# davek44/Glimmer-MG

Measured on AMD Instinct MI355X. Metric: Mbases/s scored (6-frame IMM), higher is better.
Workload: dtype f64

## Files before the change

### glimmer-mg_amd/build.py

```python
import fcntl
import os
import shutil
import subprocess

PKG = os.path.dirname(os.path.abspath(__file__))
LIB = os.path.join(PKG, "lib", "libgmg.so")
SOURCES = ["csrc/gmg_api.hip", "csrc/gmg_kernels.hip", "csrc/gmg_frame6.hip", "csrc/gmg_orfs.hip", "csrc/gmg_mg.hip", "csrc/gmg_ingest.hip", "csrc/gmg_strings.hip", "csrc/gmg_train.hip", "csrc/gmg_fixed.hip", "csrc/gmg_tophits.hip", "csrc/gmg_models.hip", "csrc/gmg_entropy.hip", "csrc/gmg_extract.hip", "csrc/gmg_features.hip", "host/icm.cc", "host/icm_train.cc", "host/fixed_icm.cc", "host/gmg_icm_c.cc", "host/gmg_shard.cc", "host/gmg_classes.cc", "host/gmg_extract_plan.cc", "host/gmg_features_host.cc"]
HEADERS = ["csrc/gmg_internal.h", "csrc/gmg_device.h", "csrc/gmg_scan.h", "csrc/gmg_mg_errtile.h", "csrc/gmg_mg_errwave.h", "csrc/gmg_mg_orfbits.h", "csrc/gmg_mg_run.h", "host/icm.hh", "host/icm_internal.hh", "../include/gmg.h", "../include/gmg_icm.h"]
FLAGS = ["--offload-arch=gfx950", "-O3", "-std=c++17", "-fPIC", "-shared", "-ffp-contract=off",
         "-Wall", "-Wno-unused-function"]


def stale():
    if not os.path.exists(LIB):
        return True
    t = os.path.getmtime(LIB)
    return any(os.path.getmtime(os.path.join(PKG, f)) > t for f in SOURCES + HEADERS)


def build_variant(name, defines):
    hipcc = shutil.which("hipcc") or "/opt/rocm/bin/hipcc"
    out = os.path.join(PKG, "lib", "variants", "libgmg_%s.so" % name)
    os.makedirs(os.path.dirname(out), exist_ok=True)
    cmd = [hipcc, *FLAGS, *["-D" + d for d in defines], "-o", out, *SOURCES]
    res = subprocess.run(cmd, cwd=PKG, stdout=subprocess.PIPE, stderr=subprocess.STDOUT, text=True)
    if res.returncode != 0:
        print(res.stdout)
        raise RuntimeError("hipcc failed building " + out)
    return out

# ... 77 lines not shown
```

### glimmer-mg_amd/capi.py

```python
import ctypes as C
import os

from .build import LIB

_lib = None

vp = C.c_void_p
u64 = C.c_uint64
i32 = C.c_int


class Segment(C.Structure):
    _fields_ = [("read", C.c_uint32), ("lo", C.c_uint32), ("len", C.c_uint32), ("orient", C.c_uint32)]


class GeneRegion(C.Structure):
    _fields_ = [("read", C.c_uint32), ("first", C.c_int32), ("len", C.c_int32), ("strand", C.c_int32)]


class Coord(C.Structure):
    _fields_ = [("read", C.c_uint32), ("dir", C.c_int32), ("start", C.c_int64), ("end", C.c_int64)]


class FeatureGene(C.Structure):
# ... 52 lines not shown
    "gmg_icm_bytes_info": (i32, [vp, u64, C.POINTER(i32), C.POINTER(i32), C.POINTER(i32), C.POINTER(i32), C.POINTER(u64)]),
    "gmg_model_set_load": (i32, [vp, vp, i32, C.POINTER(vp), vp]),
    "gmg_model_set_finish": (i32, [vp, C.POINTER(i32)]),
    "gmg_model_set_model": (vp, [vp, i32]),
    "gmg_model_set_free": (i32, [vp]),
    "gmg_model_blob": (i32, [vp, vp, C.POINTER(C.c_size_t)]),
    "gmg_model_value_stats": (i32, [vp, C.POINTER(i32), C.POINTER(i32), C.POINTER(i32)]),
    "gmg_reads_upload": (i32, [vp, vp, u64, C.POINTER(vp)]),
    "gmg_reads_wrap_device": (i32, [vp, vp, u64, u64, C.POINTER(vp)]),
    "gmg_reads_free": (i32, [vp]),
    "gmg_reads_info": (i32, [vp, C.POINTER(u64), C.POINTER(u64)]),
    "gmg_reads_download": (i32, [vp, vp, vp]),
    "gmg_reads_select": (i32, [vp, vp, u64, C.POINTER(vp)]),
    "gmg_reads_extract": (i32, [vp, vp, u64, i32, vp, vp, u64, C.POINTER(vp)]),
    "gmg_fasta_ambiguous": (i32, [C.c_char_p, u64, vp, vp, u64, C.POINTER(u64)]),
    "gmg_extract_plan": (i32, [vp, u64, vp, u64, i32, C.c_int64, vp, vp, C.POINTER(u64)]),
    "gmg_single_create": (i32, [C.POINTER(vp)]),
    "gmg_single_stage": (i32, [vp, C.c_char_p, u64, i32, C.POINTER(vp), C.POINTER(vp), C.POINTER(vp)]),
    "gmg_single_fetch": (i32, [vp, vp, C.c_size_t]),
    "gmg_single_free": (i32, [vp]),
    "gmg_single_window": (i32, [vp, vp, vp, i32, i32, vp, vp]),
    "gmg_segments_upload": (i32, [vp, vp, u64, vp, C.POINTER(u64), C.POINTER(vp)]),
    "gmg_segments_free": (i32, [vp]),
    "gmg_frame_score6": (i32, [vp, vp, vp, vp, vp]),
    "gmg_frame_score6_strided": (i32, [vp, vp, vp, vp, u64, vp]),
    "gmg_null_set_upload": (i32, [vp, i32, C.POINTER(vp)]),
    "gmg_null_set_from_tables": (i32, [vp, vp, i32, C.POINTER(vp)]),
    "gmg_null_set_build": (i32, [vp, i32, vp, i32, C.POINTER(vp)]),
    "gmg_null_set_free": (i32, [vp]),
    "gmg_frame_score6_nulls": (i32, [vp, vp, vp, vp, vp, u64, vp]),
    "gmg_segment_frame_score": (i32, [vp, vp, vp, i32, vp, vp]),
    "gmg_segment_cumscore": (i32, [vp, vp, vp, i32, vp, vp]),
    "gmg_score_string": (i32, [vp, vp, vp, i32, vp, vp]),
    "gmg_segment_partial_prob": (i32, [vp, vp, vp, i32, vp, vp]),
    "gmg_all_frame_score": (i32, [vp, vp, vp, vp, vp, vp, vp]),
    "gmg_window_distrib": (i32, [vp, vp, vp, u64, vp, vp, vp]),
    "gmg_mg_score_reads": (i32, [vp, vp, vp, vp, vp, C.POINTER(vp), vp]),
    "gmg_mg_score_groups": (i32, [vp, i32, vp, vp, vp, C.POINTER(vp), vp]),
    "gmg_find_orfs": (i32, [vp, vp, C.POINTER(vp), vp]),
    "gmg_mg_result_info": (i32, [vp, C.POINTER(u64), C.POINTER(u64)]),
    "gmg_mg_result_fetch": (i32, [vp, vp, vp, vp]),
    "gmg_mg_result_fetch_errors": (i32, [vp, vp]),
    "gmg_mg_result_free": (i32, [vp]),
    "gmg_trim_cache": (i32, []),
    "gmg_score_reads_strings": (i32, [vp, i32, vp, vp, vp]),
    "gmg_host_register": (i32, [vp, C.c_size_t]),
# ... 87 lines not shown
```

### glimmer-mg_amd/csrc/gmg_api.hip

```cpp

#include "gmg_internal.h"
#include "gmg_scan.h"

#include <ctype.h>
#include <stdarg.h>
#include <stdio.h>
#include <stdlib.h>
#include <string.h>
#include <new>
#include <mutex>
#include <vector>

static thread_local char g_err[512] = "";
static int g_device = -1;

int gmg_set_error(int code, const char *fmt, ...)
{
    va_list ap;
    va_start(ap, fmt);
    vsnprintf(g_err, sizeof g_err, fmt, ap);
    va_end(ap);
    return code;
}

extern "C" const char *gmg_last_error(void) { return g_err; }

long long g_gmg_opt[GMG_OPT_COUNT] = {
     0,  0,  0,  0,  0,  0,
     0,  -1,  0x7ffffffell,  0,  0,
     0,  0,  1,  1,  1,  1,  2,
     -1,  0,  1,  1,  0,  4,  0,  64ll << 20,  0,  0};
static const char *const g_opt_name[GMG_OPT_COUNT] = {
    "seg_plain", "mg_tile", "mg_one_stream", "mg_err_flat", "mg_err_calls", "mg_err_calls_grow", "orfs_exact_path",
    "train_sort_min", "mg_max_entries", "mg_timing", "ingest_timing", "train_timing", "diag", "strings_fused",
    "mg_gene32", "mg_fused", "mg_err_skip", "mg_orfs_events", "mg_err_tile", "mg_err_tile_q", "mg_err_qonly", "mg_err_wave", "mg_err_wave_q", "orfs_walk8", "ingest_scans", "ingest_piece_min", "mg_orfs_bits", "orfs_q_poison"};

static int opt_index(const char *key)
{
    for (int i = 0; key && i < GMG_OPT_COUNT; i++)
        if (strcmp(key, g_opt_name[i]) == 0) return i;
    return -1;
}

extern "C" int gmg_set_option(const char *key, long long value)
{
    const int i = opt_index(key);
    if (i < 0) return gmg_set_error(GMG_EINVAL, "gmg_set_option: unknown option '%s'", key ? key : "(null)");
#ifndef GMG_ABLATIONS
    if (i == GMG_OPT_DIAG && value != 0)
        return gmg_set_error(GMG_EINVAL, "gmg_set_option: the ablation kernels are not in this build (-DGMG_ABLATIONS)");
#endif
    if (i == GMG_OPT_MG_MAX_ENTRIES && (value < 1 || value > 0x7ffffffell))
        return gmg_set_error(GMG_EINVAL, "gmg_set_option: mg_max_entries must be in [1, 2^31 - 2]");
    g_gmg_opt[i] = value;
    return GMG_OK;
}

extern "C" int gmg_get_option(const char *key, long long *value)
// ... 1140 lines not shown
```

### glimmer-mg_amd/csrc/gmg_frame6.hip

```cpp

#include "gmg_device.h"
#include <stdlib.h>
#include <vector>

#ifndef GMG_F6_STAMPS
#define GMG_F6_STAMPS 0
#endif
#if GMG_F6_STAMPS
__device__ unsigned long long g_f6_stamps[1024 * 16 * 8];
extern "C" int gmg_debug_f6_stamps(unsigned long long *out, int n)
{
    return hipMemcpyFromSymbol(out, HIP_SYMBOL(g_f6_stamps), (size_t)n * 8) == hipSuccess ? 0 : -1;
}
#define F6_STAMP(i) do { const unsigned long long now_ = __builtin_readcyclecounter(); st_acc[i] += now_ - st_prev; st_prev = now_; } while (0)
#else
#define F6_STAMP(i) do { } while (0)
#endif

struct Frame6Args {
    GmgDevModel gene, nul;
    const uint32_t *packed;
    const uint64_t *off;
    const uint32_t *tile_read;
    uint64_t total, n_reads;
    uint64_t first, count;
    uint32_t p_blocks;
    double *out;
    uint64_t stride;
    float *out_gene;
    uint64_t gstride;
    double *str_sums;
    uint32_t uniform_len;
    const struct F6Round *rounds = nullptr;
    const GmgDevModel *gmodels = nullptr;
    const struct F6Range *ranges = nullptr;
    const uint64_t *group_read = nullptr;
    uint32_t n_rounds = 0, n_ranges = 0, n_groups = 0;
};
struct F6Round { uint32_t chunk0; uint32_t ng; };
#define F6_ROUND_N(r) ((r).ng & 31u)
#define F6_ROUND_GROUP(r) ((r).ng >> 5)
#define F6_MAX_GROUPS ((1 << 27) - 1)
struct F6Range { uint64_t first; uint32_t count, group; };

constexpr int f6_cstride(int dt) { return ((((1 << (2 * dt)) - 1) / 3) + 15) & ~15; }
constexpr int f6_level_base(int l) { return ((1 << (2 * l)) - 1) / 3; }

template <int CTRL, int ROW_MASK = 0xf>
__device__ __forceinline__ double f6_dpp_add(double x)
{
    const unsigned long long b = (unsigned long long)__double_as_longlong(x);
    const uint32_t lo = (uint32_t)__builtin_amdgcn_update_dpp(0, (int)(uint32_t)b, CTRL, ROW_MASK, 0xf, false);
    const uint32_t hi = (uint32_t)__builtin_amdgcn_update_dpp(0, (int)(uint32_t)(b >> 32), CTRL, ROW_MASK, 0xf, false);
    return x + __longlong_as_double((long long)((unsigned long long)hi << 32 | lo));
}
__device__ __forceinline__ double f6_row_sum(double x)
{
    x = f6_dpp_add<0xb1>(x);
    x = f6_dpp_add<0x4e>(x);
    x = f6_dpp_add<0x141>(x);
    x = f6_dpp_add<0x140>(x);
    return x;
}
__device__ __noinline__ void f6_sum_chunk_slow(double *sum, const int32_t *roff, uint32_t len, uint32_t len_magic, uint32_t rem0, int32_t wm1,
                                               uint32_t span0, uint32_t &rel_a, double f0, double r0, double f1, double r1)
{
    const uint32_t lane = threadIdx.x & 63u;
// ... 75 lines not shown
        const int32_t a0 = (int32_t)(ra * len) - (int32_t)rem0, a1 = a0 + (int32_t)len;
        if ((int32_t)span0 >= a0 + wm1 && (int32_t)span0 + 128 <= a1 - wm1) {
            rel_a = ra;
            const double f = f6_row_sum(f0 + f1), r = f6_row_sum(r0 + r1);
            if ((threadIdx.x & 15u) == 15u) { unsafeAtomicAdd(&sum[2 * ra], f); unsafeAtomicAdd(&sum[2 * ra + 1], r); }
            return;
        }
    }
    f6_sum_chunk_slow(sum, roff, len, len_magic, rem0, wm1, span0, rel_a, f0, r0, f1, r1);
}

template <int DT>
__device__ __forceinline__ uint32_t f6_descend(const uint8_t *tab, uint32_t C, uint32_t shift0)
{
    uint32_t idx = __builtin_amdgcn_ubfe(C, shift0, 2);
#pragma unroll
    for (int l = 1; l < DT; l++) {
        const uint32_t sh = tab[f6_level_base(l) + idx];
        idx = (idx << 2) | __builtin_amdgcn_ubfe(C, sh, 2);
    }
    return idx;
}

template <int BLOCK, int DT, int K, int DIAG, bool PAIR, bool GENE_ONLY, bool STRINGS = false, bool SUM = false, bool MULTI = false>
__global__ __launch_bounds__(BLOCK) void k_frame6t(Frame6Args a)
{
    constexpr int CS = f6_cstride(DT);
    constexpr uint32_t SPAN = 2 * BLOCK;
    constexpr uint32_t RAWW = SPAN / 16 + 4;
    constexpr uint32_t LEAVES = 1u << (2 * DT);
    constexpr uint32_t HALF_BYTES = LEAVES * 8;
    extern __shared__ __attribute__((aligned(16))) uint8_t s_half[];
    __shared__ __attribute__((aligned(16))) uint8_t s_shr[CS];
    __shared__ __attribute__((aligned(16))) uint8_t s_shf[CS];
    __shared__ __attribute__((aligned(16))) double s_nr[64];
    __shared__ __attribute__((aligned(16))) double s_nf[64];
    __shared__ __attribute__((aligned(16))) uint32_t s_raw[K * RAWW];
    constexpr uint32_t NR_MAX = SUM ? 384 : 1;
    __shared__ double s_sum[SUM ? 2 * NR_MAX : 1];
    __shared__ int32_t s_roff[SUM ? NR_MAX + 4 : 1];

    const uint32_t xcd = blockIdx.x & 7u, slot = blockIdx.x >> 3;
    const int ftype = STRINGS ? 0 : MULTI ? (int)((slot + xcd) % 3u) : blockIdx.x % 3;
    const uint32_t worker = STRINGS ? blockIdx.x : blockIdx.x / 3, nworkers = STRINGS ? gridDim.x : gridDim.x / 3;
    uint32_t r_lo = 0, r_step = 1, r_count = 0;
    if (MULTI) {
        auto cnt = [](uint32_t n, uint32_t c) { return n > c ? (n - c + 2u) / 3u : 0u; };
        uint32_t before = 0, total = 0, team = 0;
        for (uint32_t x = 0; x < 8; x++) {
            const uint32_t slots = (gridDim.x + 7u - x) >> 3;
            const uint32_t c = (uint32_t)(ftype + 3 * 8 - (int)x) % 3u, m = cnt(slots, c);
            if (x < xcd) before += m;
            if (x == xcd) team = m;
            total += m;
        }
        const uint32_t lo = (uint32_t)((uint64_t)a.n_rounds * before / total), hi = (uint32_t)((uint64_t)a.n_rounds * (before + team) / total);
        const uint32_t me = cnt(slot, (uint32_t)(ftype + 3 * 8 - (int)xcd) % 3u);
        r_lo = lo + me;
        r_step = team;
        r_count = hi > r_lo ? (hi - r_lo + team - 1u) / team : 0u;
    }
    const int W = a.gene.W;
    const uint8_t *half_src = (const uint8_t *)(a.gene.chalf + (size_t)ftype * 2 * LEAVES * 2);

    const uint64_t n_chunks = a.total / SPAN;
    const uint64_t per_worker = SUM ? (n_chunks + nworkers - 1) / nworkers : 0;
    const uint64_t chunk0 = SUM ? (uint64_t)worker * per_worker : worker, chunk_step = SUM ? 1 : nworkers;
    if (MULTI ? r_count == 0 : chunk0 >= n_chunks) return;
    const uint32_t n_mine = MULTI ? r_count * (uint32_t)K
                            : SUM ? (uint32_t)(n_chunks - chunk0 < per_worker ? n_chunks - chunk0 : per_worker)
                                  : (uint32_t)((n_chunks - worker + nworkers - 1) / nworkers);

    constexpr uint32_t NHALF = HALF_BYTES / 16 / BLOCK;
    const uint32_t wbase = __builtin_amdgcn_readfirstlane(threadIdx.x & ~63u);
    auto half_issue = [&](uint32_t h) __attribute__((always_inline)) {
        const float4 *src = (const float4 *)(half_src + (size_t)h * HALF_BYTES);
#pragma unroll
        for (uint32_t i = 0; i < NHALF; i++)
            __builtin_amdgcn_global_load_lds((const __attribute__((address_space(1))) void *)(src + i * BLOCK + threadIdx.x),
                                             (__attribute__((address_space(3))) void *)(s_half + (size_t)(i * BLOCK + wbase) * 16), 16, 0, 0);
    };
    auto half_landed = [&]() __attribute__((always_inline)) { __builtin_amdgcn_s_waitcnt(0x0F70); };
    constexpr uint32_t NRAW = (K * RAWW + BLOCK - 1) / BLOCK;
    uint32_t raw_t[NRAW];
    auto raw_issue = [&](uint32_t j0) __attribute__((always_inline)) {
        F6Round nd = {0, 1};
        if (MULTI) nd = a.rounds[r_lo + (j0 / K) * r_step];
#pragma unroll
        for (uint32_t i = 0; i < NRAW; i++) {
            const uint32_t t = threadIdx.x + i * BLOCK;
            const uint32_t k = t / RAWW, w = t - k * RAWW;
            const uint32_t j = j0 + k < n_mine ? j0 + k : n_mine - 1;
            const uint64_t c = MULTI ? (uint64_t)nd.chunk0 + (k < F6_ROUND_N(nd) ? k : F6_ROUND_N(nd) - 1u) : chunk0 + (uint64_t)j * chunk_step;
            raw_t[i] = t < K * RAWW ? a.packed[c * (SPAN / 16) - 1 + w] : 0u;
        }
    };
    auto raw_commit = [&]() __attribute__((always_inline)) {
#pragma unroll
        for (uint32_t i = 0; i < NRAW; i++) {
            const uint32_t t = threadIdx.x + i * BLOCK;
            if (t < K * RAWW) s_raw[t] = raw_t[i];
        }
    };

    {
        const uint8_t *sh_src = a.gene.cshift + (size_t)ftype * a.gene.cstride;
        for (int i = threadIdx.x; i < CS && !MULTI; i += BLOCK) {
            const uint8_t sh = sh_src[i];
            s_shr[i] = sh;
            s_shf[i] = (uint8_t)(2 * (W - 1) - sh);
        }
        if (threadIdx.x < 64) {
            const uint32_t i = threadIdx.x;
            const uint32_t mirrored = ((i & 3u) << 4) | (i & 12u) | (i >> 4);
            s_nr[i] = GENE_ONLY ? 0.0 : (double)a.nul.dense[(size_t)ftype * 64 + (i ^ 63u)];
            s_nf[i] = GENE_ONLY ? 0.0 : (double)a.nul.dense[(size_t)ftype * 64 + mirrored];
        }
        raw_issue(0);
        if (!MULTI) half_issue(0);
        raw_commit();
        half_landed();
    }
    __syncthreads();
    uint32_t shift0_r = MULTI ? 0u : __builtin_amdgcn_readfirstlane((uint32_t)s_shr[0]);
    uint32_t shift0_f = MULTI ? 0u : __builtin_amdgcn_readfirstlane((uint32_t)s_shf[0]);
    uint32_t cur_group = 0xffffffffu;

    const uint32_t ctx_mask = (1u << (2 * W)) - 1u;
    const uint32_t sh_f = 2u * (uint32_t)(W - 1);
    const uint32_t lane_off = 2 * threadIdx.x;
    const uint32_t first_rel = lane_off + 16u - (uint32_t)(W - 1);
    const uint32_t wword = first_rel >> 4;
    const uint32_t wsh = 2u * (first_rel & 15u);
    double *const out_f = a.out + (uint64_t)ftype * a.stride;
    double *const out_r = a.out + (uint64_t)(3 + ftype) * a.stride;

    uint64_t round_r0 = 0;
    uint32_t round_rem0 = 0, sum_rel = 0;
    const uint32_t L_u = a.uniform_len;
    const uint32_t L_magic = L_u > 1 ? (uint32_t)((0x100000000ull + L_u - 1) / L_u) : 0u;
    auto round_setup = [&](uint32_t j0) __attribute__((always_inline)) {
        const uint64_t round_g0 = (chunk0 + j0) * SPAN;
        if (L_u) {
            round_r0 = round_g0 / L_u;
            round_rem0 = (uint32_t)(round_g0 - round_r0 * L_u);
        } else {
            uint64_t r = a.tile_read[round_g0 / GMG_TILE];
            while (a.off[r + 1] <= round_g0) r++;
            round_r0 = r;
            for (uint32_t i = threadIdx.x; i < NR_MAX + 4; i += BLOCK) {
                const uint64_t rr = r + i < a.n_reads ? r + i : a.n_reads;
                const int64_t rel = (int64_t)a.off[rr] - (int64_t)round_g0;
                s_roff[i] = rel > 0x3fffffff ? 0x3fffffff : (int32_t)rel;
            }
        }
        sum_rel = 0;
        for (uint32_t i = threadIdx.x; i < 2 * NR_MAX; i += BLOCK) s_sum[i] = 0.0;
    };
// ... 51 lines not shown
                C[1] = (xl ^ flip_r) & ctx_mask;
                C[3] = (__builtin_amdgcn_alignbit(xh, xl, 2) ^ flip_r) & ctx_mask;
                C[0] = (__builtin_amdgcn_alignbit(xh, xl, sh_f) ^ flip_f) & ctx_mask;
                C[2] = (__builtin_amdgcn_alignbit(xh, xl, sh_f + 2) ^ flip_f) & ctx_mask;
                uint32_t idx[4];
                idx[0] = f6_descend<DT>(s_shf, C[0], shift0_f);
                idx[1] = f6_descend<DT>(s_shr, C[1], shift0_r);
                idx[2] = f6_descend<DT>(s_shf, C[2], shift0_f);
                idx[3] = f6_descend<DT>(s_shr, C[3], shift0_r);
                const uint32_t six = __builtin_amdgcn_alignbit(xh, xl, sh_f - 4) & 0xfffu;
#pragma unroll
                for (int b = 0; b < 2; b++) {
                    const uint32_t tf = (idx[2 * b] << 3) | ((C[2 * b] & 1u) << 2);
                    const uint32_t tr = (idx[2 * b + 1] << 3) | (((C[2 * b + 1] >> sh_f) & 1u) << 2);
                    const bool f_here = ((C[2 * b] >> 1) & 1u) == cur;
                    const uint32_t got = (DIAG & 2) ? tf : __float_as_uint(*(const float *)(s_half + (f_here ? tf : tr)));
                    have[k][b] = got;
                    want[k][b] = f_here ? tr : tf;
                }
                if (k & 1) meta[k >> 1] |= six << 16; else meta[k >> 1] = six;
            }
        }

        F6_STAMP(0);
        __syncthreads();
        F6_STAMP(1);
        cur ^= 1u;
        if (j0 + K < n_mine) raw_issue(j0 + K);
        half_issue(cur);
        if (j0 + K < n_mine) raw_commit();
        if (SUM) round_setup(j0);
        half_landed();
        F6_STAMP(2);
        __syncthreads();
        F6_STAMP(3);

#pragma unroll
        for (int k = 0; k < K; k++) {
            if ((uint32_t)k < kk) {
                const uint32_t mt = meta[k >> 1];
                const int mb = (k & 1) * 16;
                double v[4];
#pragma unroll
                for (int b = 0; b < 2; b++) {
                    const uint32_t got = (DIAG & 2) ? want[k][b] : __float_as_uint(*(const float *)(s_half + want[k][b]));
                    const uint32_t hb = (mt >> (mb + 5 + 2 * b)) & 1u;
                    const bool f_was_here = (STRINGS ? hb ^ 1u : hb) != cur;
                    const float gf = __uint_as_float(f_was_here ? have[k][b] : got);
                    const float gr = __uint_as_float(f_was_here ? got : have[k][b]);
                    if (GENE_ONLY) {
                        v[2 * b] = (double)gf;
                        v[2 * b + 1] = (double)gr;
                    } else {
                        const double nf = s_nf[__builtin_amdgcn_ubfe(mt, mb + 4 + 2 * b, 6)];
                        const double nr = s_nr[__builtin_amdgcn_ubfe(mt, mb + 2 * b, 6)];
                        v[2 * b] = (double)gf - nf;
                        v[2 * b + 1] = (double)gr - nr;
                    }
                }
                const uint64_t chunk = MULTI ? round_chunk0 + (uint64_t)k : chunk0 + (uint64_t)(j0 + k) * chunk_step;
                if (SUM) {
                    sum_chunk((uint32_t)k, v);
                } else if (GENE_ONLY) {
                    float *gf = a.out_gene + (uint64_t)(STRINGS ? 1 : ftype) * a.gstride + chunk * SPAN;
                    float *gr = a.out_gene + (uint64_t)(STRINGS ? 0 : 3 + ftype) * a.gstride + chunk * SPAN;
                    if (PAIR) {
                        typedef float f2 __attribute__((ext_vector_type(2)));
                        const f2 x0 = {(float)v[0], (float)v[2]}, x1 = {(float)v[1], (float)v[3]};
                        __builtin_nontemporal_store(x0, (f2 *)(gf + lane_off));
                        __builtin_nontemporal_store(x1, (f2 *)(gr + lane_off));
                    } else {
                        gf[lane_off] = (float)v[0]; gf[lane_off + 1] = (float)v[2];
                        gr[lane_off] = (float)v[1]; gr[lane_off + 1] = (float)v[3];
                    }
                } else if (DIAG & 1) {
                    if (v[0] + v[1] + v[2] + v[3] == 1.2345e300) a.out[lane_off] = v[0];
                } else {
                    double *pf = out_f + chunk * SPAN, *pr = out_r + chunk * SPAN;
                    if (PAIR) {
                        typedef double d2 __attribute__((ext_vector_type(2)));
                        const d2 x0 = {v[0], v[2]}, x1 = {v[1], v[3]};
                        __builtin_nontemporal_store(x0, (d2 *)(pf + lane_off));
                        __builtin_nontemporal_store(x1, (d2 *)(pr + lane_off));
                    } else {
                        __builtin_nontemporal_store(v[0], pf + lane_off);
                        __builtin_nontemporal_store(v[2], pf + lane_off + 1);
                        __builtin_nontemporal_store(v[1], pr + lane_off);
                        __builtin_nontemporal_store(v[3], pr + lane_off + 1);
                    }
                }
            }
        }
        if (SUM) {
            __syncthreads();
            round_flush();
        }
        F6_STAMP(4);
    }
#if GMG_F6_STAMPS
    if ((threadIdx.x & 63u) == 0 && blockIdx.x < 1024)
        for (int i = 0; i < 8; i++) g_f6_stamps[(blockIdx.x * 16 + (threadIdx.x >> 6)) * 8 + i] = st_acc[i];
#endif
}


__device__ __forceinline__ void f6_generic_range(const Frame6Args &a, const GmgDevModel &gene, uint64_t first, uint64_t count,
                                                 uint64_t i0, uint64_t n_lanes)
{
    for (uint64_t i = i0; i < count; i += n_lanes) {
        const uint64_t g = first + i;
        uint64_t r = a.tile_read[g / GMG_TILE];
        uint64_t r_end = a.off[r + 1];
        while (g >= r_end) { r++; r_end = a.off[r + 1]; }
        const uint64_t r_off = a.off[r];
// ... 145 lines not shown
                }
    }
    part_lo = part_hi;
    }
}

__global__ __launch_bounds__(256) void k_frame6_generic(Frame6Args a)
{
    f6_generic_range(a, (uint64_t)blockIdx.x * blockDim.x + threadIdx.x, (uint64_t)gridDim.x * blockDim.x);
}

static int launch_generic(Frame6Args a, uint64_t first, uint64_t count, hipStream_t s)
{
    if (count == 0) return GMG_OK;
    a.first = first;
    a.count = count;
    const uint64_t blocks = (count + 255) / 256;
    const unsigned grid = (unsigned)(blocks < 256 * 16 ? blocks : 256 * 16);
    hipLaunchKernelGGL(k_frame6_generic, dim3(grid), dim3(256), 0, s, a);
    GMG_HIP(hipGetLastError());
    return GMG_OK;
}

int gmg_launch_frame6(const gmg_model *gene, const gmg_model *nul, const gmg_reads *reads, double *d_out,
                      hipStream_t s)
{
    return gmg_launch_frame6_strided(gene, nul, reads, d_out, reads->total_bases, s);
}

int gmg_launch_frame6_strided(const gmg_model *gene, const gmg_model *nul, const gmg_reads *reads, double *d_out,
                              uint64_t stride, hipStream_t s)
{
    Frame6Args a;
    a.gene = gene->dev;
    a.nul = nul->dev;
    a.packed = reads->d_packed;
    a.off = reads->d_off;
    a.tile_read = reads->d_tile_read;
    a.total = reads->total_bases;
    a.n_reads = reads->n_reads;
    a.first = 0;
    a.count = 0;
    a.out = d_out;
    a.stride = stride;
    a.out_gene = nullptr;
    a.gstride = 0;
    a.str_sums = nullptr;
    a.uniform_len = 0;
    a.str_sums = nullptr;
    a.uniform_len = 0;

    const bool fast = gene->dev.has_fast && gene->dev.D == 7 && nul->dev.has_dense && nul->dev.W == 3 &&
                      gene->dev.W >= 3 && gene->dev.W <= 15;
    if (!fast) return launch_generic(a, 0, a.total, s);

    constexpr int BLOCK = 1024, DT = 7;
    constexpr uint32_t SPAN = 2 * BLOCK;
    constexpr int KR = 16;
    const uint64_t n_chunks = a.total / SPAN;
    const int diag = (int)gmg_opt(GMG_OPT_DIAG);
    const bool pair = (a.stride & 1) == 0;
    if (n_chunks > 0) {
        int dev = 0, n_cu = 256;
        GMG_HIP(hipGetDevice(&dev));
        GMG_HIP(hipDeviceGetAttribute(&n_cu, hipDeviceAttributeMultiprocessorCount, dev));
        unsigned nworkers = (unsigned)(n_cu / 3);
        if (nworkers < 1) nworkers = 1;
        if (nworkers > n_chunks) nworkers = (unsigned)n_chunks;
        const unsigned grid = 3 * nworkers;
        const size_t lds = ((size_t)1 << (2 * DT)) * 8;
#define GMG_LAUNCH_F6T(DIAG_, P_)                                                                       \
    do {                                                                                                \
        GMG_HIP(hipFuncSetAttribute((const void *)k_frame6t<BLOCK, DT, KR, DIAG_, P_, false>,           \
                                    hipFuncAttributeMaxDynamicSharedMemorySize, (int)lds));             \
        hipLaunchKernelGGL((k_frame6t<BLOCK, DT, KR, DIAG_, P_, false>), dim3(grid), dim3(BLOCK), lds, s, a); \
    } while (0)
        if (diag == 0) { if (pair) GMG_LAUNCH_F6T(0, true); else GMG_LAUNCH_F6T(0, false); }
#ifdef GMG_ABLATIONS
        else if (diag == 1 && pair) GMG_LAUNCH_F6T(1, true);
        else if (diag == 2 && pair) GMG_LAUNCH_F6T(2, true);
        else if (diag == 3 && pair) GMG_LAUNCH_F6T(3, true);
#endif
        else return gmg_set_error(GMG_EINVAL, "the ablation kernel diag=%d is not in this build", diag);
#undef GMG_LAUNCH_F6T
        GMG_HIP(hipGetLastError());
    }
    if (a.n_reads > 0) {
        const uint64_t blocks = (a.n_reads + 7) / 8;
        const unsigned grid = (unsigned)(blocks < 256 * 8 ? blocks : 256 * 8);
        const size_t lds_p = (size_t)3 * a.gene.cstride;
        a.first = n_chunks * SPAN;
        a.count = a.total - n_chunks * SPAN;
        a.p_blocks = grid;
        const unsigned tail_blocks = (unsigned)((a.count + 255) / 256);
        hipLaunchKernelGGL((k_frame6p<7, 4>), dim3(grid + tail_blocks), dim3(256), lds_p, s, a);
        GMG_HIP(hipGetLastError());
    }
    return GMG_OK;
}

static int gene6_impl(const gmg_model *gene, const gmg_reads *reads, float *d_gene, uint64_t gstride, bool full, hipStream_t s)
{
    if (!(gene->dev.has_fast && gene->dev.D == 7 && gene->dev.W >= 3 && gene->dev.W <= 15 && gene->dev.P >= 3))
        return GMG_EBADMODEL;
    Frame6Args a;
    a.gene = gene->dev;
    a.nul = gene->dev;
    a.packed = reads->d_packed;
// ... 280 lines not shown
```

### glimmer-mg_amd/csrc/gmg_internal.h

```cpp
#ifndef GMG_INTERNAL_H
#define GMG_INTERNAL_H

#include <hip/hip_runtime.h>
#include <stdint.h>
#include <vector>
#include "../../include/gmg.h"

#define GMG_MAX_MODEL_LEN 32
#define GMG_FAST_MAX_LEN 16
#define GMG_FAST_MAX_DEPTH 8
#define GMG_DENSE_MAX_LEN 6
#define GMG_TILE 1024
#define GMG_GUARD_WORDS 320

struct GmgDevModel {
    int W, D, P, N;
    const int8_t *mip;
    const float *prob;
    const uint8_t *cshift;
    const float *crow;
    const float *chalf;
    int cstride;
    int ctot;
    int has_fast;
// ... 66 lines not shown
    GMG_OPT_MG_ERR_CALLS_GROW,
    GMG_OPT_ORFS_EXACT_PATH,
    GMG_OPT_TRAIN_SORT_MIN,
    GMG_OPT_MG_MAX_ENTRIES,
    GMG_OPT_MG_TIMING,
    GMG_OPT_INGEST_TIMING,
    GMG_OPT_TRAIN_TIMING,
    GMG_OPT_DIAG,
    GMG_OPT_STRINGS_FUSED,
    GMG_OPT_MG_GENE32,
    GMG_OPT_MG_FUSED,
    GMG_OPT_MG_ERR_SKIP,
    GMG_OPT_MG_ORFS_EVENTS,
    GMG_OPT_MG_ERR_TILE,
    GMG_OPT_MG_ERR_TILE_Q,
    GMG_OPT_MG_ERR_QONLY,
    GMG_OPT_MG_ERR_WAVE,
    GMG_OPT_MG_ERR_WAVE_Q,
    GMG_OPT_ORFS_WALK8,
    GMG_OPT_INGEST_SCANS,
    GMG_OPT_INGEST_PIECE_MIN,
    GMG_OPT_MG_ORFS_BITS,
    GMG_OPT_ORFS_Q_POISON,
    GMG_OPT_COUNT
};
extern long long g_gmg_opt[GMG_OPT_COUNT];
static inline long long gmg_opt(int k) { return g_gmg_opt[k]; }

void gmg_ingest_trim(void);
hipError_t gmg_pool_alloc(void **out, size_t bytes);
void gmg_pool_release(void *p);
void gmg_pool_release_after(void *p, hipStream_t s);

struct __attribute__((visibility("hidden"))) GmgScratch {
    enum Wait { NONE, STREAM, DEVICE, AFTER };
    Wait wait = NONE;
    hipStream_t st = nullptr;
    std::vector<void *> v;
    GmgScratch() {}
    GmgScratch(Wait w, hipStream_t s) : wait(w), st(s) {}
    GmgScratch(const GmgScratch &) = delete;
    GmgScratch &operator=(const GmgScratch &) = delete;
    ~GmgScratch()
    {
        if (wait == STREAM) (void)hipStreamSynchronize(st);
        else if (wait == DEVICE) (void)hipDeviceSynchronize();
// ... 54 lines not shown
```

### include/gmg.h

```cpp
#ifndef GMG_H
#define GMG_H

#include <stddef.h>
#include <stdint.h>

#ifdef __cplusplus
extern "C" {
#endif

typedef enum gmg_status {
    GMG_OK = 0,
    GMG_EINVAL = -1,
    GMG_ENODEV = -2,
    GMG_ENOMEM = -3,
    GMG_EHIP = -4,
    GMG_EBADMODEL = -5,
    GMG_ERANGE = -6,
    GMG_ETOOBIG = -7
} gmg_status;

typedef struct gmg_model gmg_model;
typedef struct gmg_reads gmg_reads;
typedef struct gmg_segments gmg_segments;

// ... 66 lines not shown
#define GMG_COORD_SKIP_STOP 8
#define GMG_COORD_MULTI 16
int gmg_extract_plan(const uint64_t *base_offsets, uint64_t n_reads, const gmg_coord *coords, uint64_t n, int flags,
                     int64_t min_len, struct gmg_gene_region *regions, uint64_t *coord_of_region, uint64_t *n_regions);

typedef struct gmg_single gmg_single;
int gmg_single_create(gmg_single **out);
int gmg_single_stage(gmg_single *st, const char *ascii, uint64_t n, int orient, const gmg_reads **reads,
                     const gmg_segments **segs, double **d_out);
int gmg_single_fetch(gmg_single *st, double *dst, size_t n_doubles);
int gmg_single_free(gmg_single *st);
int gmg_single_window(gmg_single *st, const gmg_model *m, const uint8_t *codes, int model_len, int frame, float *dist4, double *prob);


int gmg_segments_upload(const gmg_reads *reads, const gmg_segment *segs, uint64_t n_segments,
                        uint64_t *out_offsets, uint64_t *out_total_len, gmg_segments **out);
int gmg_segments_free(gmg_segments *s);


int gmg_frame_score6(const gmg_model *gene, const gmg_model *null_model, const gmg_reads *reads,
                     double *d_out, void *stream);
int gmg_frame_score6_strided(const gmg_model *gene, const gmg_model *null_model, const gmg_reads *reads,
                             double *d_out, uint64_t row_stride, void *stream);

typedef struct gmg_null_set gmg_null_set;
int gmg_null_set_upload(const gmg_model *const *null_models, int n_models, gmg_null_set **out);
int gmg_null_set_from_tables(const int16_t *mip, const float *prob4, int n_models, gmg_null_set **out);
int gmg_null_set_build(const double *gc_frac, int n_models, const char (*stop_codon)[4], int n_stop_codons,
                       gmg_null_set **out);
int gmg_null_set_free(gmg_null_set *nulls);
int gmg_frame_score6_nulls(const gmg_model *gene, const gmg_null_set *nulls, const uint32_t *read_null,
                           const gmg_reads *reads, double *d_out, uint64_t row_stride, void *stream);

int gmg_segment_frame_score(const gmg_model *m, const gmg_reads *reads, const gmg_segments *segs,
                            int frame, double *d_out, void *stream);

int gmg_segment_cumscore(const gmg_model *m, const gmg_reads *reads, const gmg_segments *segs,
                         int frame0, double *d_out, void *stream);

int gmg_score_string(const gmg_model *m, const gmg_reads *reads, const gmg_segments *segs,
                     int frame0, double *d_sums, void *stream);

int gmg_score_reads_strings(const gmg_model *const *models, int n_models, const gmg_reads *reads,
                            double *d_sums, void *stream);

int gmg_segment_partial_prob(const gmg_model *m, const gmg_reads *reads, const gmg_segments *segs,
// ... 230 lines not shown
```

Before: 114,100.

## Add read-aligned chunk variant of 6-frame kernel with in-kernel boundary patching

For uniform-length reads, the fp64 6-frame kernel now processes chunks that hold a whole number of reads. Read-edge positions, where the context runs past a read boundary, are rescored in the kernel through a small shared-memory patch table and partial null tables. This is meant to replace the separate generic pass over read edges with a single main launch, leaving the generic kernel only for the leftover tail. It adds shared memory, a second head pass with extra branching per wave, and a host-side planner that picks reads per chunk.

Result: no change. 113,900 (-0.2%).

```diff
diff --git a/glimmer-mg_amd/build.py b/glimmer-mg_amd/build.py
--- a/glimmer-mg_amd/build.py
+++ b/glimmer-mg_amd/build.py
@@ -5,7 +5,7 @@
 
 PKG = os.path.dirname(os.path.abspath(__file__))
 LIB = os.path.join(PKG, "lib", "libgmg.so")
-SOURCES = ["csrc/gmg_api.hip", "csrc/gmg_kernels.hip", "csrc/gmg_frame6.hip", "csrc/gmg_orfs.hip", "csrc/gmg_mg.hip", "csrc/gmg_ingest.hip", "csrc/gmg_strings.hip", "csrc/gmg_train.hip", "csrc/gmg_fixed.hip", "csrc/gmg_tophits.hip", "csrc/gmg_models.hip", "csrc/gmg_entropy.hip", "csrc/gmg_extract.hip", "csrc/gmg_features.hip", "host/icm.cc", "host/icm_train.cc", "host/fixed_icm.cc", "host/gmg_icm_c.cc", "host/gmg_shard.cc", "host/gmg_classes.cc", "host/gmg_extract_plan.cc", "host/gmg_features_host.cc"]
+SOURCES = ["csrc/gmg_api.hip", "csrc/gmg_kernels.hip", "csrc/gmg_frame6.hip", "csrc/gmg_orfs.hip", "csrc/gmg_mg.hip", "csrc/gmg_ingest.hip", "csrc/gmg_strings.hip", "csrc/gmg_train.hip", "csrc/gmg_fixed.hip", "csrc/gmg_tophits.hip", "csrc/gmg_models.hip", "csrc/gmg_entropy.hip", "csrc/gmg_extract.hip", "csrc/gmg_features.hip", "host/icm.cc", "host/icm_train.cc", "host/fixed_icm.cc", "host/gmg_icm_c.cc", "host/gmg_shard.cc", "host/gmg_classes.cc", "host/gmg_extract_plan.cc", "host/gmg_features_host.cc", "host/gmg_f6_plan.cc"]
 HEADERS = ["csrc/gmg_internal.h", "csrc/gmg_device.h", "csrc/gmg_scan.h", "csrc/gmg_mg_errtile.h", "csrc/gmg_mg_errwave.h", "csrc/gmg_mg_orfbits.h", "csrc/gmg_mg_run.h", "host/icm.hh", "host/icm_internal.hh", "../include/gmg.h", "../include/gmg_icm.h"]
 FLAGS = ["--offload-arch=gfx950", "-O3", "-std=c++17", "-fPIC", "-shared", "-ffp-contract=off",
          "-Wall", "-Wno-unused-function"]
diff --git a/glimmer-mg_amd/capi.py b/glimmer-mg_amd/capi.py
--- a/glimmer-mg_amd/capi.py
+++ b/glimmer-mg_amd/capi.py
@@ -98,6 +98,7 @@
     "gmg_single_window": (i32, [vp, vp, vp, i32, i32, vp, vp]),
     "gmg_segments_upload": (i32, [vp, vp, u64, vp, C.POINTER(u64), C.POINTER(vp)]),
     "gmg_segments_free": (i32, [vp]),
+    "gmg_f6_chunk_plan": (i32, [i32, i32, i32, i32, i32]),
     "gmg_frame_score6": (i32, [vp, vp, vp, vp, vp]),
     "gmg_frame_score6_strided": (i32, [vp, vp, vp, vp, u64, vp]),
     "gmg_null_set_upload": (i32, [vp, i32, C.POINTER(vp)]),
diff --git a/glimmer-mg_amd/csrc/gmg_api.hip b/glimmer-mg_amd/csrc/gmg_api.hip
--- a/glimmer-mg_amd/csrc/gmg_api.hip
+++ b/glimmer-mg_amd/csrc/gmg_api.hip
@@ -29,11 +29,13 @@
      0,  0,  0,  0,  0,  0,
      0,  -1,  0x7ffffffell,  0,  0,
      0,  0,  1,  1,  1,  1,  2,
-     -1,  0,  1,  1,  0,  4,  0,  64ll << 20,  0,  0};
+     -1,  0,  1,  1,  0,  4,  0,  64ll << 20,  0,  0,
+     0};
 static const char *const g_opt_name[GMG_OPT_COUNT] = {
     "seg_plain", "mg_tile", "mg_one_stream", "mg_err_flat", "mg_err_calls", "mg_err_calls_grow", "orfs_exact_path",
     "train_sort_min", "mg_max_entries", "mg_timing", "ingest_timing", "train_timing", "diag", "strings_fused",
-    "mg_gene32", "mg_fused", "mg_err_skip", "mg_orfs_events", "mg_err_tile", "mg_err_tile_q", "mg_err_qonly", "mg_err_wave", "mg_err_wave_q", "orfs_walk8", "ingest_scans", "ingest_piece_min", "mg_orfs_bits", "orfs_q_poison"};
+    "mg_gene32", "mg_fused", "mg_err_skip", "mg_orfs_events", "mg_err_tile", "mg_err_tile_q", "mg_err_qonly", "mg_err_wave", "mg_err_wave_q", "orfs_walk8", "ingest_scans", "ingest_piece_min", "mg_orfs_bits", "orfs_q_poison",
+    "f6_two_launch"};
 
 static int opt_index(const char *key)
 {
diff --git a/glimmer-mg_amd/csrc/gmg_frame6.hip b/glimmer-mg_amd/csrc/gmg_frame6.hip
--- a/glimmer-mg_amd/csrc/gmg_frame6.hip
+++ b/glimmer-mg_amd/csrc/gmg_frame6.hip
@@ -31,6 +31,7 @@
     uint64_t gstride;
     double *str_sums;
     uint32_t uniform_len;
+    uint32_t al_reads = 0;
     const struct F6Round *rounds = nullptr;
     const GmgDevModel *gmodels = nullptr;
     const struct F6Range *ranges = nullptr;
@@ -43,6 +44,7 @@
 #define F6_MAX_GROUPS ((1 << 27) - 1)
 struct F6Range { uint64_t first; uint32_t count, group; };
 
+#define F6_PATCH_BYTES 8192
 constexpr int f6_cstride(int dt) { return ((((1 << (2 * dt)) - 1) / 3) + 15) & ~15; }
 constexpr int f6_level_base(int l) { return ((1 << (2 * l)) - 1) / 3; }
 
@@ -164,9 +166,11 @@
     return idx;
 }
 
-template <int BLOCK, int DT, int K, int DIAG, bool PAIR, bool GENE_ONLY, bool STRINGS = false, bool SUM = false, bool MULTI = false>
+template <int BLOCK, int DT, int K, int DIAG, bool PAIR, bool GENE_ONLY, bool STRINGS = false, bool SUM = false, bool MULTI = false,
+          bool ALIGNED = false>
 __global__ __launch_bounds__(BLOCK) void k_frame6t(Frame6Args a)
 {
+    static_assert(!ALIGNED || (PAIR && !GENE_ONLY && !STRINGS && !SUM && !MULTI && DIAG == 0), "read-aligned chunks: the fp64 table only");
     constexpr int CS = f6_cstride(DT);
     constexpr uint32_t SPAN = 2 * BLOCK;
     constexpr uint32_t RAWW = SPAN / 16 + 4;
@@ -175,12 +179,14 @@
     extern __shared__ __attribute__((aligned(16))) uint8_t s_half[];
     __shared__ __attribute__((aligned(16))) uint8_t s_shr[CS];
     __shared__ __attribute__((aligned(16))) uint8_t s_shf[CS];
-    __shared__ __attribute__((aligned(16))) double s_nr[64];
-    __shared__ __attribute__((aligned(16))) double s_nf[64];
+    constexpr int NULLS = ALIGNED ? 192 : 64;
+    __shared__ __attribute__((aligned(16))) double s_nr[NULLS];
+    __shared__ __attribute__((aligned(16))) double s_nf[NULLS];
     __shared__ __attribute__((aligned(16))) uint32_t s_raw[K * RAWW];
     constexpr uint32_t NR_MAX = SUM ? 384 : 1;
     __shared__ double s_sum[SUM ? 2 * NR_MAX : 1];
     __shared__ int32_t s_roff[SUM ? NR_MAX + 4 : 1];
+    __shared__ float s_patch[ALIGNED ? F6_PATCH_BYTES / 4 : 1];
 
     const uint32_t xcd = blockIdx.x & 7u, slot = blockIdx.x >> 3;
     const int ftype = STRINGS ? 0 : MULTI ? (int)((slot + xcd) % 3u) : blockIdx.x % 3;
@@ -205,7 +211,9 @@
     const int W = a.gene.W;
     const uint8_t *half_src = (const uint8_t *)(a.gene.chalf + (size_t)ftype * 2 * LEAVES * 2);
 
-    const uint64_t n_chunks = a.total / SPAN;
+    const uint32_t CB = ALIGNED ? a.al_reads * a.uniform_len : SPAN;
+    const uint32_t HZ = 2u * (uint32_t)(W - 1), HRZ = a.al_reads * HZ;
+    const uint64_t n_chunks = ALIGNED ? a.n_reads / a.al_reads : a.total / SPAN;
     const uint64_t per_worker = SUM ? (n_chunks + nworkers - 1) / nworkers : 0;
     const uint64_t chunk0 = SUM ? (uint64_t)worker * per_worker : worker, chunk_step = SUM ? 1 : nworkers;
     if (MULTI ? r_count == 0 : chunk0 >= n_chunks) return;
@@ -234,7 +242,7 @@
             const uint32_t k = t / RAWW, w = t - k * RAWW;
             const uint32_t j = j0 + k < n_mine ? j0 + k : n_mine - 1;
             const uint64_t c = MULTI ? (uint64_t)nd.chunk0 + (k < F6_ROUND_N(nd) ? k : F6_ROUND_N(nd) - 1u) : chunk0 + (uint64_t)j * chunk_step;
-            raw_t[i] = t < K * RAWW ? a.packed[c * (SPAN / 16) - 1 + w] : 0u;
+            raw_t[i] = t < K * RAWW && (!ALIGNED || w < CB / 16 + 4) ? a.packed[c * (CB / 16) - 1 + w] : 0u;
         }
     };
     auto raw_commit = [&]() __attribute__((always_inline)) {
@@ -257,6 +265,13 @@
             const uint32_t mirrored = ((i & 3u) << 4) | (i & 12u) | (i >> 4);
             s_nr[i] = GENE_ONLY ? 0.0 : (double)a.nul.dense[(size_t)ftype * 64 + (i ^ 63u)];
             s_nf[i] = GENE_ONLY ? 0.0 : (double)a.nul.dense[(size_t)ftype * 64 + mirrored];
+            if (ALIGNED) {
+                const float *np = a.nul.dense_part + (size_t)ftype * a.nul.n_dense_part;
+                s_nr[64 + i] = (double)np[(i >> 4) ^ 3u];
+                s_nr[128 + i] = (double)np[4u + ((i >> 2) ^ 15u)];
+                s_nf[64 + i] = (double)np[i & 3u];
+                s_nf[128 + i] = (double)np[4u + (((i & 3u) << 2) | ((i >> 2) & 3u))];
+            }
         }
         raw_issue(0);
         if (!MULTI) half_issue(0);
@@ -276,6 +291,23 @@
     const uint32_t wsh = 2u * (first_rel & 15u);
     double *const out_f = a.out + (uint64_t)ftype * a.stride;
     double *const out_r = a.out + (uint64_t)(3 + ftype) * a.stride;
+
+    uint32_t hpk[2] = {0u, 0u};
+    bool head_wave = false;
+    const float *const crow_f = a.gene.crow + (size_t)ftype * a.gene.ctot * 4;
+    if (ALIGNED) {
+#pragma unroll
+        for (int b = 0; b < 2; b++) {
+            const uint32_t pos = lane_off + b;
+            const uint32_t q = pos / a.uniform_len, e = pos - q * a.uniform_len;
+            if (pos < CB && e < (uint32_t)(W - 1)) hpk[b] = (q * HZ + e) | 1u << 9 | (e < 2u ? e + 1u : 0u) << 12;
+            if (pos < CB && e + (uint32_t)(W - 1) >= a.uniform_len) {
+                const uint32_t j = a.uniform_len - 1u - e;
+                hpk[b] = (q * HZ + (uint32_t)(W - 1) + j) | 1u << 8 | (j < 2u ? j + 1u : 0u) << 10;
+            }
+        }
+        head_wave = __builtin_amdgcn_ballot_w64((hpk[0] | hpk[1]) != 0u) != 0;
+    }
 
     uint64_t round_r0 = 0;
     uint32_t round_rem0 = 0, sum_rel = 0;
@@ -373,6 +405,44 @@
             }
         }
 
+        float hv[2] = {0.0f, 0.0f};
+        if (ALIGNED) {
+            F6_STAMP(5);
+            const uint32_t n_items = (uint32_t)K * HRZ;
+#pragma unroll
+            for (int t = 0; t < 2; t++) {
+                const uint32_t task = (threadIdx.x >> 6) + (uint32_t)(BLOCK / 64) * t;
+                if (task * 64u < n_items) {
+                    uint32_t item = task * 64u + (threadIdx.x & 63u);
+                    asm volatile("" : "+v"(item));
+                    const bool live = item < n_items;
+                    if (!live) item = 0;
+                    const uint32_t k = item / HRZ, rem = item - k * HRZ;
+                    const uint32_t q = rem / HZ, z = rem - q * HZ;
+                    const bool rev = z >= (uint32_t)(W - 1);
+                    const uint32_t j = rev ? z - (uint32_t)(W - 1) : z;
+                    const uint32_t pos = q * a.uniform_len + (rev ? a.uniform_len - 1u - j : j);
+                    const uint32_t frel = pos + 16u - (uint32_t)(W - 1);
+                    const uint32_t *w = s_raw + k * RAWW + (frel >> 4);
+                    const uint32_t w0 = w[0], w1 = w[1], w2 = w[2], ws = 2u * (frel & 15u);
+                    const uint32_t xl = __builtin_amdgcn_alignbit(w1, w0, ws), xh = __builtin_amdgcn_alignbit(w2, w1, ws);
+                    const uint32_t C = rev ? __builtin_amdgcn_alignbit(xh, xl, sh_f) & ctx_mask : (xl ^ ctx_mask) & ctx_mask;
+                    const uint8_t *tab = rev ? s_shf : s_shr;
+                    const uint32_t thr2 = 2u * ((uint32_t)(W - 1) - j);
+                    uint32_t idx = 0, node = 0xffffffffu;
+#pragma unroll
+                    for (int l = 0; l < DT; l++) {
+                        const uint32_t sh = tab[f6_level_base(l) + idx];
+                        if (node == 0xffffffffu && (rev ? sh_f - sh : sh) < thr2) node = f6_level_base(l) + idx;
+                        idx = (idx << 2) | __builtin_amdgcn_ubfe(C, sh, 2);
+                    }
+                    if (node == 0xffffffffu) node = f6_level_base(DT) + idx;
+                    const uint32_t pred = rev ? C & 3u : (C >> sh_f) & 3u;
+                    hv[t] = crow_f[live ? node << 2 | pred : 0u];
+                }
+            }
+        }
+
         F6_STAMP(0);
         __syncthreads();
         F6_STAMP(1);
@@ -382,16 +452,38 @@
         if (j0 + K < n_mine) raw_commit();
         if (SUM) round_setup(j0);
         half_landed();
+        if (ALIGNED) {
+#pragma unroll
+            for (int t = 0; t < 2; t++) {
+                const uint32_t item = threadIdx.x + (uint32_t)BLOCK * t;
+                if (item < (uint32_t)K * HRZ) s_patch[item] = hv[t];
+            }
+        }
         F6_STAMP(2);
         __syncthreads();
         F6_STAMP(3);
 
+#pragma unroll
+        for (int pass = 0; pass < (ALIGNED ? 2 : 1); pass++) {
+        const bool HEADS = pass == 1;
+        if (ALIGNED && (lane_off >= CB || head_wave != HEADS)) continue;
+        uint32_t hp[2] = {hpk[0], hpk[1]};
+        if (ALIGNED) asm volatile("" : "+v"(hp[0]), "+v"(hp[1]));
+        const uint32_t ppo[2] = {hp[0] & 0xffu, hp[1] & 0xffu};
+        const bool hd_f[2] = {(hp[0] & 0x100u) != 0, (hp[1] & 0x100u) != 0}, hd_r[2] = {(hp[0] & 0x200u) != 0, (hp[1] & 0x200u) != 0};
+        const uint32_t nfr[2] = {(hp[0] >> 10 & 3u) << 9, (hp[1] >> 10 & 3u) << 9}, nrr[2] = {(hp[0] >> 12 & 3u) << 9, (hp[1] >> 12 & 3u) << 9};
+        auto uni64 = [](uint64_t x) __attribute__((always_inline)) {
+            return (uint64_t)__builtin_amdgcn_readfirstlane((uint32_t)(x >> 32)) << 32 | __builtin_amdgcn_readfirstlane((uint32_t)x);
+        };
+        const uint64_t al_step = ALIGNED ? uni64((uint64_t)chunk_step * CB) : 0;
+        uint64_t al_base = ALIGNED ? uni64((chunk0 + (uint64_t)j0 * chunk_step) * CB) : 0;
 #pragma unroll
         for (int k = 0; k < K; k++) {
             if ((uint32_t)k < kk) {
                 const uint32_t mt = meta[k >> 1];
                 const int mb = (k & 1) * 16;
                 double v[4];
+                if (!ALIGNED) {
 #pragma unroll
                 for (int b = 0; b < 2; b++) {
                     const uint32_t got = (DIAG & 2) ? want[k][b] : __float_as_uint(*(const float *)(s_half + want[k][b]));
@@ -409,12 +501,46 @@
                         v[2 * b + 1] = (double)gr - nr;
                     }
                 }
+                } else {
+                float gf[2], gr[2];
+#pragma unroll
+                for (int b = 0; b < 2; b++) {
+                    const uint32_t got = __float_as_uint(*(const float *)(s_half + want[k][b]));
+                    const bool f_was_here = ((mt >> (mb + 5 + 2 * b)) & 1u) != cur;
+                    gf[b] = __uint_as_float(f_was_here ? have[k][b] : got);
+                    gr[b] = __uint_as_float(f_was_here ? got : have[k][b]);
+                }
+                if (HEADS) {
+#pragma unroll
+                    for (int b = 0; b < 2; b++) {
+                        const float pv = s_patch[(uint32_t)k * HRZ + ppo[b]];
+                        gf[b] = hd_f[b] ? pv : gf[b];
+                        gr[b] = hd_r[b] ? pv : gr[b];
+                    }
+                }
+#pragma unroll
+                for (int b = 0; b < 2; b++) {
+                    if (HEADS) {
+                        const double nf = *(const double *)((const uint8_t *)s_nf + ((__builtin_amdgcn_ubfe(mt, mb + 4 + 2 * b, 6) << 3) + nfr[b]));
+                        const double nr = *(const double *)((const uint8_t *)s_nr + ((__builtin_amdgcn_ubfe(mt, mb + 2 * b, 6) << 3) + nrr[b]));
+                        v[2 * b] = (double)gf[b] - nf;
+                        v[2 * b + 1] = (double)gr[b] - nr;
+                    } else {
+                        const double nf = s_nf[__builtin_amdgcn_ubfe(mt, mb + 4 + 2 * b, 6)];
+                        const double nr = s_nr[__builtin_amdgcn_ubfe(mt, mb + 2 * b, 6)];
+                        v[2 * b] = (double)gf[b] - nf;
+                        v[2 * b + 1] = (double)gr[b] - nr;
+                    }
+                }
+                }
                 const uint64_t chunk = MULTI ? round_chunk0 + (uint64_t)k : chunk0 + (uint64_t)(j0 + k) * chunk_step;
+                const uint64_t cbase = ALIGNED ? al_base : chunk * SPAN;
+                if (ALIGNED) al_base += al_step;
                 if (SUM) {
                     sum_chunk((uint32_t)k, v);
                 } else if (GENE_ONLY) {
-                    float *gf = a.out_gene + (uint64_t)(STRINGS ? 1 : ftype) * a.gstride + chunk * SPAN;
-                    float *gr = a.out_gene + (uint64_t)(STRINGS ? 0 : 3 + ftype) * a.gstride + chunk * SPAN;
+                    float *gf = a.out_gene + (uint64_t)(STRINGS ? 1 : ftype) * a.gstride + cbase;
+                    float *gr = a.out_gene + (uint64_t)(STRINGS ? 0 : 3 + ftype) * a.gstride + cbase;
                     if (PAIR) {
                         typedef float f2 __attribute__((ext_vector_type(2)));
                         const f2 x0 = {(float)v[0], (float)v[2]}, x1 = {(float)v[1], (float)v[3]};
@@ -427,7 +553,7 @@
                 } else if (DIAG & 1) {
                     if (v[0] + v[1] + v[2] + v[3] == 1.2345e300) a.out[lane_off] = v[0];
                 } else {
-                    double *pf = out_f + chunk * SPAN, *pr = out_r + chunk * SPAN;
+                    double *pf = out_f + cbase, *pr = out_r + cbase;
                     if (PAIR) {
                         typedef double d2 __attribute__((ext_vector_type(2)));
                         const d2 x0 = {v[0], v[2]}, x1 = {v[1], v[3]};
@@ -441,6 +567,7 @@
                     }
                 }
             }
+        }
         }
         if (SUM) {
             __syncthreads();
@@ -632,6 +759,13 @@
     return GMG_OK;
 }
 
+static uint32_t f6_aligned_reads(const gmg_reads *reads, int W, int K, uint64_t row_stride)
+{
+    if (reads->uniform_len <= 0 || (row_stride & 1) || gmg_opt(GMG_OPT_F6_TWO_LAUNCH)) return 0;
+    if ((uint64_t)reads->uniform_len * reads->n_reads != reads->total_bases) return 0;
+    return (uint32_t)gmg_f6_chunk_plan(reads->uniform_len, W, K, 2048, F6_PATCH_BYTES);
+}
+
 int gmg_launch_frame6(const gmg_model *gene, const gmg_model *nul, const gmg_reads *reads, double *d_out,
                       hipStream_t s)
 {
@@ -667,9 +801,15 @@
     constexpr int BLOCK = 1024, DT = 7;
     constexpr uint32_t SPAN = 2 * BLOCK;
     constexpr int KR = 16;
-    const uint64_t n_chunks = a.total / SPAN;
+    uint64_t n_chunks = a.total / SPAN;
     const int diag = (int)gmg_opt(GMG_OPT_DIAG);
     const bool pair = (a.stride & 1) == 0;
+    const uint32_t al = diag == 0 ? f6_aligned_reads(reads, gene->dev.W, KR, a.stride) : 0;
+    if (al) {
+        a.al_reads = al;
+        a.uniform_len = (uint32_t)reads->uniform_len;
+        n_chunks = a.n_reads / al;
+    }
     if (n_chunks > 0) {
         int dev = 0, n_cu = 256;
         GMG_HIP(hipGetDevice(&dev));
@@ -685,7 +825,11 @@
                                     hipFuncAttributeMaxDynamicSharedMemorySize, (int)lds));             \
         hipLaunchKernelGGL((k_frame6t<BLOCK, DT, KR, DIAG_, P_, false>), dim3(grid), dim3(BLOCK), lds, s, a); \
     } while (0)
-        if (diag == 0) { if (pair) GMG_LAUNCH_F6T(0, true); else GMG_LAUNCH_F6T(0, false); }
+        if (al) {
+            GMG_HIP(hipFuncSetAttribute((const void *)k_frame6t<BLOCK, DT, KR, 0, true, false, false, false, false, true>,
+                                        hipFuncAttributeMaxDynamicSharedMemorySize, (int)lds));
+            hipLaunchKernelGGL((k_frame6t<BLOCK, DT, KR, 0, true, false, false, false, false, true>), dim3(grid), dim3(BLOCK), lds, s, a);
+        } else if (diag == 0) { if (pair) GMG_LAUNCH_F6T(0, true); else GMG_LAUNCH_F6T(0, false); }
 #ifdef GMG_ABLATIONS
         else if (diag == 1 && pair) GMG_LAUNCH_F6T(1, true);
         else if (diag == 2 && pair) GMG_LAUNCH_F6T(2, true);
@@ -694,6 +838,10 @@
         else return gmg_set_error(GMG_EINVAL, "the ablation kernel diag=%d is not in this build", diag);
 #undef GMG_LAUNCH_F6T
         GMG_HIP(hipGetLastError());
+    }
+    if (al) {
+        const uint64_t done = n_chunks * al * a.uniform_len;
+        return launch_generic(a, done, a.total - done, s);
     }
     if (a.n_reads > 0) {
         const uint64_t blocks = (a.n_reads + 7) / 8;
diff --git a/glimmer-mg_amd/csrc/gmg_internal.h b/glimmer-mg_amd/csrc/gmg_internal.h
--- a/glimmer-mg_amd/csrc/gmg_internal.h
+++ b/glimmer-mg_amd/csrc/gmg_internal.h
@@ -112,6 +112,7 @@
     GMG_OPT_INGEST_PIECE_MIN,
     GMG_OPT_MG_ORFS_BITS,
     GMG_OPT_ORFS_Q_POISON,
+    GMG_OPT_F6_TWO_LAUNCH,
     GMG_OPT_COUNT
 };
 extern long long g_gmg_opt[GMG_OPT_COUNT];
diff --git a/glimmer-mg_amd/host/gmg_f6_plan.cc b/glimmer-mg_amd/host/gmg_f6_plan.cc
--- /dev/null
+++ b/glimmer-mg_amd/host/gmg_f6_plan.cc
@@ -0,0 +1,18 @@
+
+#include "../../include/gmg.h"
+
+#include <stdint.h>
+
+extern "C" int gmg_f6_chunk_plan(int L, int W, int K, int span, int patch_bytes)
+{
+    if (L < 1 || W < 2 || K < 1 || span < 16 || patch_bytes < 1 || L > span) return 0;
+    if (L < 2 * (W - 1)) return 0;
+    for (int R = span / L; R >= 1; R--) {
+        const int64_t bases = (int64_t)R * L;
+        if (bases % 16 != 0) continue;
+        if (bases < span - span / 16) break;
+        if ((int64_t)K * R * 2 * (W - 1) * 4 > patch_bytes) continue;
+        return R;
+    }
+    return 0;
+}
diff --git a/include/gmg.h b/include/gmg.h
--- a/include/gmg.h
+++ b/include/gmg.h
@@ -112,6 +112,7 @@
                      double *d_out, void *stream);
 int gmg_frame_score6_strided(const gmg_model *gene, const gmg_model *null_model, const gmg_reads *reads,
                              double *d_out, uint64_t row_stride, void *stream);
+int gmg_f6_chunk_plan(int L, int W, int K, int span, int patch_bytes);
 
 typedef struct gmg_null_set gmg_null_set;
 int gmg_null_set_upload(const gmg_model *const *null_models, int n_models, gmg_null_set **out);
```
